# sarahappleby/VAMP

Measured on AMD Instinct MI355X. Metric: walker-steps/sec (log-posterior evals/sec), higher is better.
Workload: dtype f64

## Files before the change

__graft_entry__.py:

```python
import os
import subprocess
import sys

ROOT = os.path.dirname(os.path.abspath(__file__))
if ROOT not in sys.path:
    sys.path.insert(0, ROOT)


def build() -> None:
    from vamp_amd import build as vb
    vb.build()
    subprocess.check_call(["make", "-C", os.path.join(ROOT, "oracle"), "-s"])
    host = os.path.join(ROOT, "tests", "host")
    so = os.path.join(host, "libvoigt_host.so")
    src = os.path.join(host, "voigt_host.cpp")
    hdr = os.path.join(ROOT, "vamp_amd", "csrc", "voigt_math.hpp")
    if not os.path.exists(so) or os.path.getmtime(so) < max(os.path.getmtime(src), os.path.getmtime(hdr)):
        subprocess.check_call(["g++", "-O2", "-std=c++17", "-shared", "-fPIC", "-ffp-contract=off", "-o", so, src])
    pso, psrc = os.path.join(host, "libff_pred_host.so"), os.path.join(host, "ff_pred_host.cpp")
    phdr = os.path.join(ROOT, "vamp_amd", "csrc", "ff_predicates.hpp")
    if not os.path.exists(pso) or os.path.getmtime(pso) < max(os.path.getmtime(psrc), os.path.getmtime(phdr), os.path.getmtime(hdr)):
        subprocess.check_call(["g++", "-O2", "-std=c++17", "-shared", "-fPIC", "-ffp-contract=off", "-o", pso, psrc])
    oso, osrc = os.path.join(host, "libnp_order_host.so"), os.path.join(host, "np_order_host.cpp")
    if not os.path.exists(oso) or os.path.getmtime(oso) < max(os.path.getmtime(osrc), os.path.getmtime(phdr), os.path.getmtime(hdr)):
        subprocess.check_call(["g++", "-O2", "-std=c++17", "-shared", "-fPIC", "-ffp-contract=off", "-o", oso, osrc])
    fake, fsrc = os.path.join(host, "librccl_fake.so"), os.path.join(host, "rccl_fake.cpp")
    if not os.path.exists(fake) or os.path.getmtime(fake) < os.path.getmtime(fsrc):
        subprocess.check_call([os.environ.get("HIPCC", "/opt/rocm/bin/hipcc"), "-O1", "-std=c++17", "-shared", "-fPIC", "-o", fake, fsrc, "-lrt"])
    import vamp_amd
    os.environ.setdefault("VAMP_NO_IMPORT_ORDER_WARNING", "1")
    vamp_amd._lib.load()


def smoke() -> None:
    import numpy as np
    import torch

    import vamp_amd
    from oracle import vamp_oracle as vo

# ... 48 lines not shown
```

vamp_amd/build.py:

```python
import os
import subprocess
import sys

HERE = os.path.dirname(os.path.abspath(__file__))
SRC = os.path.join(HERE, "csrc", "vamp_hip.hip")
OUT = os.path.join(HERE, "libvamp_hip.so")
DEPS = [SRC] + [os.path.join(HERE, "csrc", f) for f in ("ff_matrix.inc", "ff_matrix32.inc", "voigt_math.hpp", "map_search.hpp", "host_plan.hpp",
                                                         "abi_state.hpp", "draws.hpp", "ff_predicates.hpp", "ff_moments.hpp")
                if os.path.exists(os.path.join(HERE, "csrc", f))] + [os.path.join(HERE, "..", "include", "vamp_hip.h")]


FLAGS = ["--offload-arch=gfx950", "-O3", "-std=c++17", "-fno-slp-vectorize", "-shared", "-fPIC"]

SIDE_FLAGS = ["--offload-arch=gfx950", "-O3", "-std=c++17", "-shared", "-fPIC", "-fvisibility=hidden"]
POST_FLAGS = EVID_FLAGS = PRED_FLAGS = LOO_FLAGS = RELABEL_FLAGS = SIDE_FLAGS
SIDE_CALL = os.path.join(HERE, "csrc", "side_call.hpp")
LANE_GROUP = os.path.join(HERE, "csrc", "lane_group.hpp")
CHAIN_GROUPS = os.path.join(HERE, "csrc", "chain_groups.hpp")

DIAG_SRC = os.path.join(HERE, "csrc", "chain_diag.hip")
DIAG_OUT = os.path.join(HERE, "libvamp_diag.so")
DIAG_DEPS = [DIAG_SRC, SIDE_CALL, os.path.join(HERE, "..", "include", "vamp_diag.h")]

POST_SRC = os.path.join(HERE, "csrc", "posterior.hip")
# ... 72 lines not shown
```

vamp_amd/csrc/ff_predicates.hpp:

```cpp
#pragma once
#include "voigt_math.hpp"

namespace vamp {

constexpr double FF_ZONE_MARGIN = 1.0 / 1024.0;

VAMP_DEV bool ff_tile_in_zone(double c, double s, double y, double mid, double half) {
    const double Xf = (fabs(mid - c) + half) * s;
    return fma(Xf, Xf, y * y) < R2_CORE * (1.0 - FF_ZONE_MARGIN);
}

struct NpOrder {
    unsigned long long seq;
    unsigned solo;
    int pairs[4];
};
VAMP_DEV NpOrder np_pair_order(unsigned far, unsigned n6, unsigned n4, unsigned n3) {
    NpOrder o;
    const unsigned cls[4] = {n6, n4 & ~n6, n3 & ~n4, far & ~n3};
    unsigned long long seq = 0ull;
    int sh = 0, last = 0;
    for (int c = 0; c < 4; ++c) {
        for (unsigned m = cls[c]; m; m &= m - 1u) {
            last = __builtin_ctz(m);
// ... 16 lines not shown
```

vamp_amd/csrc/vamp_hip.hip:

```cpp
#include <hip/hip_runtime.h>
#include <dlfcn.h>

#include <algorithm>
#include <atomic>
#include <chrono>
#include <cmath>
#include <cstdint>
#include <cstdio>
#include <cstdlib>
#include <cstring>
#include <new>
#include <string>
#include <vector>

#include "../../include/vamp_hip.h"
#include "abi_state.hpp"
#include "draws.hpp"
#include "host_plan.hpp"
#include "map_search.hpp"
#include "voigt_math.hpp"
#include "ff_predicates.hpp"
#include "ff_moments.hpp"

#ifndef VAMP_EARLY_LOADS
// ... 52 lines not shown
#endif
#ifndef VAMP_WIDE_MAX
#define VAMP_WIDE_MAX 0.75
#endif
#ifndef VAMP_F32_LEAN_STAGE
#define VAMP_F32_LEAN_STAGE 1
#endif
#ifndef VAMP_TILE_MOMENTS
#define VAMP_TILE_MOMENTS 2
#endif
#ifndef VAMP_NODE_PASS
#define VAMP_NODE_PASS 1
#endif
#ifndef VAMP_NP_CLASS_RUNS
#define VAMP_NP_CLASS_RUNS 1
#endif
#ifndef VAMP_TAB_PAIR
#define VAMP_TAB_PAIR 0
#endif
#ifndef VAMP_TILE_HEAD
#define VAMP_TILE_HEAD 0
#endif
namespace {

constexpr int KMAX = 16;
constexpr int KMAX_ALL = VAMP_MAX_COMPONENTS;
static_assert(KMAX_ALL >= KMAX && KMAX_ALL < 64, "lane k stages line k; one spare lane for sd");
constexpr int WAVES_PER_BLOCK = 4;
constexpr long long PACK_MIN_WALKERS = 16384;
constexpr int RES_MAX_MOVERS = 128;
// ... 966 lines not shown
    }
    }
}

#if VAMP_NODE_PASS && VAMP_TILE_MOMENTS != 1 && !VAMP_X_PREFETCH && !defined(VAMP_SKIP_NEAR) && !defined(VAMP_SKIP_FFNODES) && \
    !defined(VAMP_SKIP_CLENSHAW) && !defined(VAMP_SKIP_EXP)
#define VAMP_NODE_PASS_ON 1
#else
#define VAMP_NODE_PASS_ON 0
#endif
#if VAMP_NODE_PASS_ON
__device__ __forceinline__ unsigned ff_fold16(unsigned long long m) {
    const unsigned h = (unsigned)m | (unsigned)(m >> 32);
    return (h | (h >> 16)) & 0xffffu;
}
struct NodeSets { unsigned far, n6, n4, n3, wide; };
template <bool WIDE, bool ZONE, class LDS>
__device__ __forceinline__ void ff_classify_batch_np(const LDS& L, const double2* __restrict__ geo, int K, int lane_, int base, int stride,
                                                     unsigned wide_all, unsigned long long& farmasks, unsigned long long& widemasks,
                                                     unsigned long long& zonemasks, NodeSets& sets, double& mid, double& half) {
    int lane = lane_;
    asm volatile("" : "+v"(lane));
    const int j = lane >> 4, k = lane & (KMAX - 1);
    const double2 g = geo[(base + j * stride) >> 8];
    mid = g.x, half = fabs(g.y);
    const LineRec& me = *reinterpret_cast<const LineRec*>(reinterpret_cast<const char*>(L.line) +
                                                          __umul24((unsigned)(k < K ? k : 0), (unsigned)sizeof(LineRec)));
    const double my_c = me.c, my_s = me.s, my_y = me.y, my_w8 = me.w8, my_wmid = me.wmid;
    const double dist = fabs(mid - my_c) - half;
    const bool my_beyond = (k < K) & (dist >= FF_DIST * half);
    const bool my_far = my_beyond & (dist >= my_w8);
    const double Xe = dist * my_s, r2e = fma(Xe, Xe, my_y * my_y);
    farmasks = __ballot(my_far);
    sets.far = ff_fold16(farmasks);
    sets.n6 = ff_fold16(__ballot(my_far & (r2e < VAMP_FF_R2_M4)));
    sets.n4 = ff_fold16(__ballot(my_far & (r2e < VAMP_FF_R2_M3)));
    sets.n3 = ff_fold16(__ballot(my_far & (r2e < VAMP_FF_R2_M2)));
    widemasks = 0ull;
    if constexpr (WIDE) {
        const bool my_wide = ((((wide_all >> k) & 1u) != 0u) | (VAMP_MID_NODES && (my_beyond & (dist >= my_wmid)))) & !my_far;
        widemasks = __ballot(my_wide);
    }
    sets.wide = ff_fold16(widemasks);
    zonemasks = 0ull;
    if constexpr (ZONE) zonemasks = __ballot(vamp::ff_tile_in_zone(my_c, my_s, my_y, mid, half));
}
constexpr double FF_X_IDLE = 64.0;
static_assert(FF_X_IDLE * FF_X_IDLE >= VAMP_FF_R2_M2 && FF_X_IDLE < vamp::X_FAR, "the idle argument neither deepens a pair nor needs a guard");
template <int M> struct NpDepth { static constexpr int value = M; };
template <bool WIDE, bool GUARD, class LDS>
__device__ __forceinline__ double ff_node_pass(const LDS& L, const double* __restrict__ dct, const double* tab, int lane_, double mid, double half,
                                               unsigned long long farmasks, unsigned long long widemasks, NodeSets sets) {
    int lane = lane_;
    asm volatile("" : "+v"(lane));
    const double xnode = fma(half, dct[FF_MAT + (lane & (FF_NODES - 1))], mid);
    const unsigned far16 = ff_tile_field(farmasks, lane);
    double fs = 0.0;
#if VAMP_NP_CLASS_RUNS
    if (sets.far != 0u) {
    const vamp::NpOrder ord = vamp::np_pair_order(sets.far, sets.n6, sets.n4, sets.n3);
    unsigned long long seq = ord.seq;
    const unsigned far16b = far16 & ~ord.solo;
    struct Pair { double c[2], s[2], y[2], amp[2]; };
    auto read_pair = [&](unsigned long long q) {
        Pair p;
#pragma unroll
        for (int t = 0; t < 2; ++t) {
            const LineRec& ln = L.line[(unsigned)(q >> (4 * t)) & 15u];
            p.c[t] = ln.c, p.s[t] = ln.s, p.y[t] = ln.y, p.amp[t] = ln.amp;
        }
        return p;
    };
// ... 120 lines not shown
                                                        double& chi) {
    if ((lane >> 4) == j) Sx.coef[lane & (FF_NODES - 1)] = a_row;
    const int n = lane & (FF_NODES - 1), g4 = (lane >> 4) * 4;
    const double2* Qr = reinterpret_cast<const double2*>(mt + vamp::FFN_Q + n * FF_NODES + g4);
    const double2 q01 = Qr[0], q23 = Qr[1];
    const double Sv = mt[vamp::FFN_S + n];
    __builtin_amdgcn_wave_barrier();
    const double2* av = reinterpret_cast<const double2*>(Sx.coef + g4);
    const double2 a01 = av[0], a23 = av[1];
    const double a = Sx.coef[n];
    const double acc0 = fma(q01.x, a01.x, 0.5 * Sv), acc1 = q01.y * a01.y;
    const double term = a * (fma(q23.x, a23.x, acc0) + fma(q23.y, a23.y, acc1));
    chi += lane == 0 ? term + c0 : term;
    __builtin_amdgcn_wave_barrier();
}
template <int MODE, class PK, bool TAB, bool WIDE = false, bool GUARD = true>
__device__ __forceinline__ void sweep_range_ff_np(const RegionDev& R, const typename PK::Lds& L, TileScratch& Sx, const double* __restrict__ dct,
                                                  const double* __restrict__ x, const double* __restrict__ f,
                                                  const double* __restrict__ wt, const double* __restrict__ ut,
                                                  const double2* __restrict__ geo, int lane, int base0, int base1, int stride,
                                                  double& chi, const double* tab, unsigned long long wide_all = 0ull,
                                                  const double* __restrict__ mom = nullptr) {
    constexpr int T = TPIX;
    static_assert(PK::LPW == 64 && PK::KCAP <= 16, "far-field tiles: one walker per wavefront, <= 16 lines");
    const int K = R.K;
    const int ntile = base0 < base1 ? (base1 - base0 + stride - 1) / stride : 0;
    const int bfull = __builtin_amdgcn_readfirstlane(base0 + (ntile / FF_BATCH) * (FF_BATCH * stride));
    for (int batch = __builtin_amdgcn_readfirstlane(base0); batch < bfull; batch += FF_BATCH * stride) {
    unsigned long long farmasks, widemasks, zonemasks;
    double fsn;
    {
        NodeSets sets;
        double mid_j, half_j;
        ff_classify_batch_np<WIDE, TAB>(L, geo, K, lane, batch, stride, (unsigned)wide_all, farmasks, widemasks, zonemasks, sets, mid_j, half_j);
        fsn = ff_node_pass<WIDE, GUARD>(L, dct, tab, lane, mid_j, half_j, farmasks, widemasks, sets);
    }
#if VAMP_TILE_MOMENTS == 2
    {
        unsigned long long fm = farmasks, wm = widemasks;
        double a_row = 0.0, amax_row = 0.0;
        bool have_a = false;
#pragma unroll 1
        for (int j = 0; j < FF_BATCH; ++j, fm >>= KMAX, wm >>= KMAX) {
            const unsigned farmask = (unsigned)fm & 0xffffu, widemask = WIDE ? (unsigned)wm & 0xffffu : 0u;
            if ((~(farmask | widemask) & ((1u << K) - 1u)) != 0u) continue;
            const double* mt = mom + ((batch + j * stride) >> 8) * MOM_TILE;
            const double root_c0 = mt[MOM_RC], root_q0 = mt[MOM_RQ];
            if (!vamp::ff_moments_try(root_c0, root_q0)) continue;
            if (!have_a) {
                int eoff = FF_EXP;
                asm volatile("" : "+s"(eoff));
                a_row = -vamp::expm1_taylor_tab(-fsn, dct + eoff);
                amax_row = row16_max(fabs(a_row));
                have_a = true;
            }
            const double amax = __hiloint2double(__builtin_amdgcn_readlane(__double2hiint(amax_row), KMAX * j),
                                                 __builtin_amdgcn_readlane(__double2loint(amax_row), KMAX * j));
            if (!vamp::ff_moments_ok(root_c0, root_q0, amax)) continue;
            ff_moment_chi_nodes_row(Sx, mt, lane_here(), j, a_row, mt[vamp::FFN_C0], chi);
            const unsigned long long field = 0xffffull << (KMAX * j);
            farmasks |= field;
            widemasks |= field;
        }
    }
#endif
#pragma unroll 1
    for (int j = 0; j < FF_BATCH; ++j, farmasks >>= KMAX, widemasks >>= KMAX, zonemasks >>= KMAX) {
        const int base = batch + j * stride;
        double xi[T], tau[T];
#if VAMP_TILE_HEAD
        if ((unsigned)farmasks & (unsigned)widemasks & 0xffffu) continue;
#endif
#pragma unroll
        for (int t = 0; t < T; ++t) {
            xi[t] = x[base + 64 * t + lane];
            tau[t] = 0.0;
        }
#if !VAMP_TILE_HEAD
        if ((unsigned)farmasks & (unsigned)widemasks & 0xffffu) continue;
#endif
        const bool up = __double2hiint(geo[base >> 8].y) >= 0;
        const unsigned farmask = (unsigned)farmasks & 0xffffu;
        const unsigned widemask = WIDE ? (unsigned)widemasks & 0xffffu : 0u;
// ... 39 lines not shown
        int eoff = FF_EXP;
        asm volatile("" : "+s"(eoff));
        const double* ec = dct + eoff;
#pragma unroll
        for (int t = 0; t < T; ++t) {
#if !VAMP_EARLY_LOADS
            fi[t] = f[base + 64 * t + lane];
            wi[t] = wt[base + 64 * t + lane];
#endif
            const double m = vamp::exp_taylor_tab<VAMP_FLUX_EXP_DROP>(-tau[t], ec);
            const double r = (fi[t] - m) * wi[t];
            chi = fma(r, r, chi);
        }
    }
    }
    if (bfull < base1) sweep_range_ff<MODE, PK, TAB, WIDE, GUARD>(R, L, Sx, dct, x, f, wt, ut, geo, lane, bfull, base1, stride, chi, tab, wide_all, mom);
}
#endif
template <int MODE, class PK, bool TAB, bool WIDE, bool GUARD, class... Args>
__device__ __forceinline__ void sweep_range_ff_any(Args&&... args) {
#if VAMP_NODE_PASS_ON
    sweep_range_ff_np<MODE, PK, TAB, WIDE, GUARD>(static_cast<Args&&>(args)...);
#else
    sweep_range_ff<MODE, PK, TAB, WIDE, GUARD>(static_cast<Args&&>(args)...);
#endif
}

#ifndef VAMP_FARFIELD
#define VAMP_FARFIELD 1
#endif

template <int T, int LPW = 64>
__device__ __forceinline__ void tile_w4(float y, const float (&X)[T], float (&H)[T]) {
    float lo = X[0];
#pragma unroll
    for (int t = 1; t < T; ++t) lo = fminf(lo, X[t]);
    lo += y;
// ... 365 lines not shown
                    sweep_range_f32<MODE, PK, 1>(R, L, x, f, wt, lane, from, R.P, PK::LPW, chi);
                }
            }
    } else {
        const double* x = px.x + R.pix_off; const double* f = px.f + R.pix_off; const double* wt = px.wt + R.pix_off;
        if constexpr (VAMP_FARFIELD && PK::FF && MODE != VAMP_GAUSS3 && TPIX == 4) {
            const double* ut = px.u + R.pix_off;
            const double2* geo = px.geo + (R.pix_off >> 8);
            const double* mom = VAMP_TILE_MOMENTS ? px.mom + (R.pix_off >> 8) * MOM_TILE : nullptr;
            const int flags = __builtin_amdgcn_readfirstlane((int)(__double_as_longlong(L.theta[4 * PK::KCAP + 2]) & 0x3ffff));
            const bool guard = (flags >> 16) != 0;
            if constexpr (VAMP_WIDE_NODES && TAB) {
                const unsigned long long wide_all = (unsigned long long)(flags & 0xffff);
                if (VAMP_MID_NODES || wide_all) {
                    if (guard) sweep_range_ff_any<MODE, PK, TAB, true, true>(R, L, Sx, dct, x, f, wt, ut, geo, lane, base0, full, stride, chi, tab, wide_all, mom);
                    else sweep_range_ff_any<MODE, PK, TAB, true, false>(R, L, Sx, dct, x, f, wt, ut, geo, lane, base0, full, stride, chi, tab, wide_all, mom);
                } else {
                    if (guard) sweep_range_ff_any<MODE, PK, TAB, false, true>(R, L, Sx, dct, x, f, wt, ut, geo, lane, base0, full, stride, chi, tab, 0ull, mom);
                    else sweep_range_ff_any<MODE, PK, TAB, false, false>(R, L, Sx, dct, x, f, wt, ut, geo, lane, base0, full, stride, chi, tab, 0ull, mom);
                }
            } else {
                if (guard) sweep_range_ff_any<MODE, PK, TAB, false, true>(R, L, Sx, dct, x, f, wt, ut, geo, lane, base0, full, stride, chi, tab, 0ull, mom);
                else sweep_range_ff_any<MODE, PK, TAB, false, false>(R, L, Sx, dct, x, f, wt, ut, geo, lane, base0, full, stride, chi, tab, 0ull, mom);
            }
        } else if (TPIX > 1) sweep_range<MODE, PK, TPIX, TAB>(R, L, x, f, wt, lane, base0, full, stride, chi, tab);
        if constexpr (PK::TAIL || TPIX == 1)
            if (tail) {
                const int from = TPIX > 1 ? full : 0;
                if constexpr (!PK::FF && TPIX > 1) {
                    const int nt = (R.P - from + PK::LPW - 1) / PK::LPW;
                    if constexpr (TPIX >= 4) { if (nt == 4) sweep_range<MODE, PK, 4, TAB>(R, L, x, f, wt, lane, from, from + 1, 1 << 28, chi, tab); }
                    if constexpr (TPIX >= 3) { if (nt == 3) sweep_range<MODE, PK, 3, TAB>(R, L, x, f, wt, lane, from, from + 1, 1 << 28, chi, tab); }
                    if (nt == 2) sweep_range<MODE, PK, 2, TAB>(R, L, x, f, wt, lane, from, from + 1, 1 << 28, chi, tab);
                    else if (nt == 1) sweep_range<MODE, PK, 1, TAB>(R, L, x, f, wt, lane, from, from + 1, 1 << 28, chi, tab);
                } else {
                    sweep_range<MODE, PK, 1, TAB>(R, L, x, f, wt, lane, from, R.P, PK::LPW, chi, tab);
                }
            }
// ... 235 lines not shown
        for (int d = l; d < R.D; d += PK::LPW) L.theta[d] = theta[w * R.D + d];
    group_barrier<PK>();
    double chi;
    const double v = wave_lnprob<F32, MODE, PK>(R, L, scr[PK::FF ? wave : 0], dct, px, l, &chi, wave, red,
                                                tabs[PK::SPLIT ? 0 : wave].a);
    if (PK::SPLIT && wave != 0) return;
    if (l == 0) {
        lnprob[w] = v;
        if (chi2) chi2[w] = chi;
    }
}

template <int MODE>
__global__ __launch_bounds__(PackSplit::THREADS) void k_dbg_node_sums(const RegionDev* __restrict__ regions, int region, PixPtrs px,
                                                                      const double* __restrict__ theta, double* __restrict__ nodes,
                                                                      unsigned* __restrict__ sets_out) {
    using PK = PackSplit;
    __shared__ typename PK::Lds lds[1];
    __shared__ TileScratch scr[PK::WPB];
    __shared__ alignas(16) double dct[ff_table_doubles<false>()];
    __shared__ LineTables<table_doubles<false, MODE, PK>()> tabs[1];
    ff_fill_table<false>(dct);
    const int wave = threadIdx.x >> 6, lane = threadIdx.x & 63;
    const RegionDev R = regions[region];
    typename PK::Lds& L = lds[0];
    if (wave == 0)
        for (int d = lane; d < R.D; d += 64) L.theta[d] = theta[d];
    group_barrier<PK>();
    const double lp = stage_lines<MODE, PK, true, false, false, true>(R, L, lane, false, wave, tabs[0].a, px.x + R.pix_off);
    if (!(lp > NEG_INF)) return;
    TileScratch& Sx = scr[wave];
    const double* tab = tabs[0].a;
    const double2* geo = px.geo + (R.pix_off >> 8);
    const int flags = __builtin_amdgcn_readfirstlane((int)(__double_as_longlong(L.theta[4 * PK::KCAP + 2]) & 0x3ffff));
    const bool guard = (flags >> 16) != 0;
    const unsigned wide_all = (unsigned)(flags & 0xffff);
    constexpr int TILE = 64 * TPIX;
    const int K = R.K, base1 = (R.P / TILE) * TILE, stride = PARTS * TILE;
    const int base0 = __builtin_amdgcn_readfirstlane(wave * TILE);
    int bfull = base0;
#if VAMP_NODE_PASS_ON
    const int ntile = base0 < base1 ? (base1 - base0 + stride - 1) / stride : 0;
    bfull = __builtin_amdgcn_readfirstlane(base0 + (ntile / FF_BATCH) * (FF_BATCH * stride));
    for (int batch = base0; batch < bfull; batch += FF_BATCH * stride) {
        unsigned long long farmasks, widemasks, zonemasks;
        NodeSets sets;
        double mid, half;
        ff_classify_batch_np<true, true>(L, geo, K, lane, batch, stride, wide_all, farmasks, widemasks, zonemasks, sets, mid, half);
        const double fs = guard ? ff_node_pass<true, true>(L, dct, tab, lane, mid, half, farmasks, widemasks, sets)
                                : ff_node_pass<true, false>(L, dct, tab, lane, mid, half, farmasks, widemasks, sets);
        nodes[((batch + (lane >> 4) * stride) >> 8) * FF_NODES + (lane & (FF_NODES - 1))] = fs;
        if (lane == 0) {
            unsigned* so = sets_out + (batch >> 8) * 5;
            so[0] = sets.far, so[1] = sets.n6, so[2] = sets.n4, so[3] = sets.n3, so[4] = sets.wide;
        }
    }
#endif
    for (int batch = bfull; batch < base1; batch += FF_BATCH * stride) {
        unsigned long long farmasks, widemasks, zonemasks;
        ff_classify_batch<true, false, true>(L, Sx, geo, K, lane, batch, base1, stride, wide_all, farmasks, widemasks, zonemasks);
        for (int j = 0; j < FF_BATCH; ++j, farmasks >>= KMAX, widemasks >>= KMAX) {
            const int base = batch + j * stride;
            if (base >= base1) break;
            const double2 tg = geo[base >> 8];
            const double mid = tg.x, half = fabs(tg.y);
            const int nfar = __builtin_popcount((unsigned)farmasks & 0xffffu), nwide = __builtin_popcount((unsigned)widemasks & 0xffffu);
            const double fs_wide = nwide > 0 ? ff_wide_nodes<typename PK::Lds>(L, Sx.widelist[j], dct, tab, lane, nwide, mid, half) : 0.0;
            const double fs = guard ? ff_node_sums<typename PK::Lds, true>(L, Sx.farlist[j], dct, lane, nfar, mid, half, fs_wide)
                                    : ff_node_sums<typename PK::Lds, false>(L, Sx.farlist[j], dct, lane, nfar, mid, half, fs_wide);
            if (lane < FF_NODES) nodes[(base >> 8) * FF_NODES + lane] = fs;
        }
        __builtin_amdgcn_wave_barrier();
    }
// ... 1204 lines not shown
    HIP_TRY(hipMemcpy(geo_out, c->geo_d.get(), slots * sizeof(double2), hipMemcpyDeviceToHost));
    return slots;
}

long long vampdbg_tile_moments(vamp_ctx* c, double* out) {
    if (!c) return fail(VAMP_ERR_ARG, "vampdbg_tile_moments: bad argument");
    if (c->regions_h.empty()) return fail(VAMP_ERR_STATE, "vampdbg_tile_moments: call vamp_set_regions first");
    if (!VAMP_TILE_MOMENTS || c->f32 || !c->geo_d || !c->mom_d) return 0;
    const long long N = c->regions_h.back().pix_off + c->regions_h.back().P;
    const long long slots = N / (64 * TPIX) + 1;
    HIP_TRY(hipStreamSynchronize(c->stream));
    if (out) HIP_TRY(hipMemcpy(out, c->mom_d.get(), slots * MOM_TILE * sizeof(double), hipMemcpyDeviceToHost));
    return MOM_TILE;
}

long long vampdbg_node_sums(vamp_ctx* c, int region, const double* theta, double* nodes, unsigned* sets) {
    if (!c || !theta || !nodes || !sets) return fail(VAMP_ERR_ARG, "vampdbg_node_sums: bad argument");
    if (c->regions_h.empty()) return fail(VAMP_ERR_STATE, "vampdbg_node_sums: call vamp_set_regions first");
    if (region < 0 || region >= c->n_regions) return fail(VAMP_ERR_ARG, "vampdbg_node_sums: no such region");
    const RegionDev& R = c->regions_h[region];
    const long long tiles = R.P / (64 * TPIX);
    if (c->f32 || c->mode == VAMP_GAUSS3 || !c->geo_d || tiles == 0 || R.K > KMAX) return 0;
    HIP_TRY(hipSetDevice(c->device));
    DevBuf<double> th_d, nodes_d;
    DevBuf<unsigned> sets_d;
    HIP_TRY(th_d.ensure(R.D));
    HIP_TRY(nodes_d.ensure(tiles * FF_NODES));
    HIP_TRY(sets_d.ensure(tiles * 5));
    HIP_TRY(hipMemcpy(th_d.get(), theta, R.D * sizeof(double), hipMemcpyHostToDevice));
    HIP_TRY(hipMemset(nodes_d.get(), 0, tiles * FF_NODES * sizeof(double)));
    HIP_TRY(hipMemset(sets_d.get(), 0xff, tiles * 5 * sizeof(unsigned)));
    HIP_TRY(hipStreamSynchronize(c->stream));
    if (c->mode == VAMP_VOIGT4)
        hipLaunchKernelGGL((k_dbg_node_sums<VAMP_VOIGT4>), dim3(1), dim3(PackSplit::THREADS), 0, c->stream, c->regions_d.get(), region, c->pix(),
                           th_d.get(), nodes_d.get(), sets_d.get());
    else
        hipLaunchKernelGGL((k_dbg_node_sums<VAMP_NBZ3>), dim3(1), dim3(PackSplit::THREADS), 0, c->stream, c->regions_d.get(), region, c->pix(),
                           th_d.get(), nodes_d.get(), sets_d.get());
    HIP_TRY(hipGetLastError());
    HIP_TRY(hipStreamSynchronize(c->stream));
    HIP_TRY(hipMemcpy(nodes, nodes_d.get(), tiles * FF_NODES * sizeof(double), hipMemcpyDeviceToHost));
    HIP_TRY(hipMemcpy(sets, sets_d.get(), tiles * 5 * sizeof(unsigned), hipMemcpyDeviceToHost));
    return tiles;
}

int vamp_version(void) { return VAMP_ABI_VERSION; }

const char* vamp_last_error(void) { return vamp::last_error().c_str(); }

int vamp_device_count(int* n) {
    if (int rc = vamp::check_device_count(n)) return rc;
    HIP_TRY(hipGetDeviceCount(n));
    return VAMP_OK;
}

int vamp_ctx_create(vamp_ctx** out, int device, int dtype, int wofz_kind) {
    if (int rc = vamp::check_ctx_create(out, dtype, wofz_kind)) return rc;
    int ndev = 0;
// ... 642 lines not shown
```

Baseline: 13.75 million.

## Deal adjacent tiles per wave batch and add optional super-tile node pass

Batches in the node pass now cover adjacent tiles rather than tiles strided across waves, with a remainder sweep for leftovers. This groups neighbouring tiles so their line classifications and geometry are similar and can be shared. It also adds a compile-time-disabled super-node pass that evaluates distant lines once on a merged super-tile using a DCT/Chebyshev expansion. The adjacent dealing changes per-wave work distribution and may hurt load balance across waves.

```diff
diff --git a/__graft_entry__.py b/__graft_entry__.py
--- a/__graft_entry__.py
+++ b/__graft_entry__.py
@@ -24,6 +24,10 @@
     oso, osrc = os.path.join(host, "libnp_order_host.so"), os.path.join(host, "np_order_host.cpp")
     if not os.path.exists(oso) or os.path.getmtime(oso) < max(os.path.getmtime(osrc), os.path.getmtime(phdr), os.path.getmtime(hdr)):
         subprocess.check_call(["g++", "-O2", "-std=c++17", "-shared", "-fPIC", "-ffp-contract=off", "-o", oso, osrc])
+    sso, ssrc = os.path.join(host, "libsuper_nodes_host.so"), os.path.join(host, "super_nodes_host.cpp")
+    sinc = os.path.join(ROOT, "vamp_amd", "csrc", "ff_super.inc")
+    if not os.path.exists(sso) or os.path.getmtime(sso) < max(os.path.getmtime(ssrc), os.path.getmtime(phdr), os.path.getmtime(hdr), os.path.getmtime(sinc)):
+        subprocess.check_call(["g++", "-O2", "-std=c++17", "-shared", "-fPIC", "-ffp-contract=off", "-o", sso, ssrc])
     fake, fsrc = os.path.join(host, "librccl_fake.so"), os.path.join(host, "rccl_fake.cpp")
     if not os.path.exists(fake) or os.path.getmtime(fake) < os.path.getmtime(fsrc):
         subprocess.check_call([os.environ.get("HIPCC", "/opt/rocm/bin/hipcc"), "-O1", "-std=c++17", "-shared", "-fPIC", "-o", fake, fsrc, "-lrt"])
diff --git a/vamp_amd/build.py b/vamp_amd/build.py
--- a/vamp_amd/build.py
+++ b/vamp_amd/build.py
@@ -6,7 +6,7 @@
 SRC = os.path.join(HERE, "csrc", "vamp_hip.hip")
 OUT = os.path.join(HERE, "libvamp_hip.so")
 DEPS = [SRC] + [os.path.join(HERE, "csrc", f) for f in ("ff_matrix.inc", "ff_matrix32.inc", "voigt_math.hpp", "map_search.hpp", "host_plan.hpp",
-                                                         "abi_state.hpp", "draws.hpp", "ff_predicates.hpp", "ff_moments.hpp")
+                                                         "abi_state.hpp", "draws.hpp", "ff_predicates.hpp", "ff_moments.hpp", "ff_super.inc")
                 if os.path.exists(os.path.join(HERE, "csrc", f))] + [os.path.join(HERE, "..", "include", "vamp_hip.h")]
 
 
diff --git a/vamp_amd/csrc/ff_predicates.hpp b/vamp_amd/csrc/ff_predicates.hpp
--- a/vamp_amd/csrc/ff_predicates.hpp
+++ b/vamp_amd/csrc/ff_predicates.hpp
@@ -8,6 +8,48 @@
 VAMP_DEV bool ff_tile_in_zone(double c, double s, double y, double mid, double half) {
     const double Xf = (fabs(mid - c) + half) * s;
     return fma(Xf, Xf, y * y) < R2_CORE * (1.0 - FF_ZONE_MARGIN);
+}
+
+#ifndef VAMP_SUPER_DIST
+#define VAMP_SUPER_DIST 4.0
+#endif
+#ifndef VAMP_FF_R2_M3
+#define VAMP_FF_R2_M3 300.0
+#endif
+VAMP_DEV bool ff_super_distant(double c, double s, double y, double Mid, double Half) {
+    const double distS = fabs(Mid - c) - Half;
+    const double Xe = distS * s;
+    return (distS >= VAMP_SUPER_DIST * Half) & (fma(Xe, Xe, y * y) >= VAMP_FF_R2_M3);
+}
+VAMP_DEV double ff_super_r2e(double c, double s, double y, double Mid, double Half) {
+    const double Xe = (fabs(Mid - c) - Half) * s;
+    return fma(Xe, Xe, y * y);
+}
+VAMP_DEV void ff_super_tile(double mid0, double half0, double mid3, double half3, double& Mid, double& Half) {
+    const double lo = fmin(mid0 - half0, mid3 - half3), hi = fmax(mid0 + half0, mid3 + half3);
+    Mid = 0.5 * (lo + hi);
+    Half = 0.5 * (hi - lo);
+}
+
+struct SuperOrder {
+    unsigned long long seq;
+    int n, iters, iters3;
+};
+VAMP_DEV SuperOrder super_order(unsigned dist, unsigned d3) {
+    SuperOrder o;
+    const unsigned cls[2] = {d3 & dist, dist & ~d3};
+    unsigned long long seq = 0ull;
+    int sh = 0;
+    for (int c = 0; c < 2; ++c)
+        for (unsigned m = cls[c]; m; m &= m - 1u) {
+            seq |= (unsigned long long)__builtin_ctz(m) << sh;
+            sh += 4;
+        }
+    o.seq = seq;
+    o.n = sh >> 2;
+    o.iters = (o.n + 7) >> 3;
+    o.iters3 = (__builtin_popcount(cls[0]) + 7) >> 3;
+    return o;
 }
 
 struct NpOrder {
diff --git a/vamp_amd/csrc/ff_super.inc b/vamp_amd/csrc/ff_super.inc
--- /dev/null
+++ b/vamp_amd/csrc/ff_super.inc
@@ -0,0 +1,133 @@
+#ifndef FF_SUPER_QUAL
+#define FF_SUPER_QUAL __device__
+#endif
+FF_SUPER_QUAL const double FF_SUPER_C[256] = {
+    6.25000000000000000e-02, 6.25000000000000000e-02,
+    1.24398090834024616e-01, 1.19617541966526103e-01,
+    1.22598160050403804e-01, 1.03933701537818154e-01,
+    1.19617541966526103e-01, 7.92991605204556860e-02,
+    1.15484941563910842e-01, 4.78354290456362227e-02,
+    1.10240158043544381e-01, 1.22521425411950755e-02,
+    1.03933701537818154e-01, -2.43862902520160345e-02,
+    9.66263066703421242e-02, -5.89245921032497053e-02,
+    8.83883476483184466e-02, -8.83883476483184466e-02,
+    7.92991605204556860e-02, -1.10240158043544381e-01,
+    6.94462791274502722e-02, -1.22598160050403804e-01,
+    5.89245921032497053e-02, -1.24398090834024616e-01,
+    4.78354290456362227e-02, -1.15484941563910842e-01,
+    3.62855846568077983e-02, -9.66263066703421242e-02,
+    2.43862902520160345e-02, -6.94462791274502722e-02,
+    1.22521425411950755e-02, -3.62855846568077983e-02,
+    6.25000000000000000e-02, 6.25000000000000000e-02,
+    1.10240158043544381e-01, 9.66263066703421242e-02,
+    6.94462791274502722e-02, 2.43862902520160345e-02,
+    1.22521425411950755e-02, -5.89245921032497053e-02,
+    -4.78354290456362227e-02, -1.15484941563910842e-01,
+    -9.66263066703421242e-02, -1.19617541966526103e-01,
+    -1.22598160050403804e-01, -6.94462791274502722e-02,
+    -1.19617541966526103e-01, 1.22521425411950755e-02,
+    -8.83883476483184466e-02, 8.83883476483184466e-02,
+    -3.62855846568077983e-02, 1.24398090834024616e-01,
+    2.43862902520160345e-02, 1.03933701537818154e-01,
+    7.92991605204556860e-02, 3.62855846568077983e-02,
+    1.15484941563910842e-01, -4.78354290456362227e-02,
+    1.24398090834024616e-01, -1.10240158043544381e-01,
+    1.03933701537818154e-01, -1.22598160050403804e-01,
+    5.89245921032497053e-02, -7.92991605204556860e-02,
+    6.25000000000000000e-02, 6.25000000000000000e-02,
+    7.92991605204556860e-02, 5.89245921032497053e-02,
+    -2.43862902520160345e-02, -6.94462791274502722e-02,
+    -1.10240158043544381e-01, -1.24398090834024616e-01,
+    -1.15484941563910842e-01, -4.78354290456362227e-02,
+    -3.62855846568077983e-02, 7.92991605204556860e-02,
+    6.94462791274502722e-02, 1.22598160050403804e-01,
+    1.24398090834024616e-01, 3.62855846568077983e-02,
+    8.83883476483184466e-02, -8.83883476483184466e-02,
+    -1.22521425411950755e-02, -1.19617541966526103e-01,
+    -1.03933701537818154e-01, -2.43862902520160345e-02,
+    -1.19617541966526103e-01, 9.66263066703421242e-02,
+    -4.78354290456362227e-02, 1.15484941563910842e-01,
+    5.89245921032497053e-02, 1.22521425411950755e-02,
+    1.22598160050403804e-01, -1.03933701537818154e-01,
+    9.66263066703421242e-02, -1.10240158043544381e-01,
+    6.25000000000000000e-02, 6.25000000000000000e-02,
+    3.62855846568077983e-02, 1.22521425411950755e-02,
+    -1.03933701537818154e-01, -1.22598160050403804e-01,
+    -9.66263066703421242e-02, -3.62855846568077983e-02,
+    4.78354290456362227e-02, 1.15484941563910842e-01,
+    1.24398090834024616e-01, 5.89245921032497053e-02,
+    2.43862902520160345e-02, -1.03933701537818154e-01,
+    -1.10240158043544381e-01, -7.92991605204556860e-02,
+    -8.83883476483184466e-02, 8.83883476483184466e-02,
+    5.89245921032497053e-02, 9.66263066703421242e-02,
+    1.22598160050403804e-01, -6.94462791274502722e-02,
+    1.22521425411950755e-02, -1.10240158043544381e-01,
+    -1.15484941563910842e-01, 4.78354290456362227e-02,
+    -7.92991605204556860e-02, 1.19617541966526103e-01,
+    6.94462791274502722e-02, -2.43862902520160345e-02,
+    1.19617541966526103e-01, -1.24398090834024616e-01,
+    6.25000000000000000e-02, 6.25000000000000000e-02,
+    -1.22521425411950755e-02, -3.62855846568077983e-02,
+    -1.22598160050403804e-01, -1.03933701537818154e-01,
+    3.62855846568077983e-02, 9.66263066703421242e-02,
+    1.15484941563910842e-01, 4.78354290456362227e-02,
+    -5.89245921032497053e-02, -1.24398090834024616e-01,
+    -1.03933701537818154e-01, 2.43862902520160345e-02,
+    7.92991605204556860e-02, 1.10240158043544381e-01,
+    8.83883476483184466e-02, -8.83883476483184466e-02,
+    -9.66263066703421242e-02, -5.89245921032497053e-02,
+    -6.94462791274502722e-02, 1.22598160050403804e-01,
+    1.10240158043544381e-01, -1.22521425411950755e-02,
+    4.78354290456362227e-02, -1.15484941563910842e-01,
+    -1.19617541966526103e-01, 7.92991605204556860e-02,
+    -2.43862902520160345e-02, 6.94462791274502722e-02,
+    1.24398090834024616e-01, -1.19617541966526103e-01,
+    6.25000000000000000e-02, 6.25000000000000000e-02,
+    -5.89245921032497053e-02, -7.92991605204556860e-02,
+    -6.94462791274502722e-02, -2.43862902520160345e-02,
+    1.24398090834024616e-01, 1.10240158043544381e-01,
+    -4.78354290456362227e-02, -1.15484941563910842e-01,
+    -7.92991605204556860e-02, 3.62855846568077983e-02,
+    1.22598160050403804e-01, 6.94462791274502722e-02,
+    -3.62855846568077983e-02, -1.24398090834024616e-01,
+    -8.83883476483184466e-02, 8.83883476483184466e-02,
+    1.19617541966526103e-01, 1.22521425411950755e-02,
+    -2.43862902520160345e-02, -1.03933701537818154e-01,
+    -9.66263066703421242e-02, 1.19617541966526103e-01,
+    1.15484941563910842e-01, -4.78354290456362227e-02,
+    -1.22521425411950755e-02, -5.89245921032497053e-02,
+    -1.03933701537818154e-01, 1.22598160050403804e-01,
+    1.10240158043544381e-01, -9.66263066703421242e-02,
+    6.25000000000000000e-02, 6.25000000000000000e-02,
+    -9.66263066703421242e-02, -1.10240158043544381e-01,
+    2.43862902520160345e-02, 6.94462791274502722e-02,
+    5.89245921032497053e-02, -1.22521425411950755e-02,
+    -1.15484941563910842e-01, -4.78354290456362227e-02,
+    1.19617541966526103e-01, 9.66263066703421242e-02,
+    -6.94462791274502722e-02, -1.22598160050403804e-01,
+    -1.22521425411950755e-02, 1.19617541966526103e-01,
+    8.83883476483184466e-02, -8.83883476483184466e-02,
+    -1.24398090834024616e-01, 3.62855846568077983e-02,
+    1.03933701537818154e-01, 2.43862902520160345e-02,
+    -3.62855846568077983e-02, -7.92991605204556860e-02,
+    -4.78354290456362227e-02, 1.15484941563910842e-01,
+    1.10240158043544381e-01, -1.24398090834024616e-01,
+    -1.22598160050403804e-01, 1.03933701537818154e-01,
+    7.92991605204556860e-02, -5.89245921032497053e-02,
+    6.25000000000000000e-02, 6.25000000000000000e-02,
+    -1.19617541966526103e-01, -1.24398090834024616e-01,
+    1.03933701537818154e-01, 1.22598160050403804e-01,
+    -7.92991605204556860e-02, -1.19617541966526103e-01,
+    4.78354290456362227e-02, 1.15484941563910842e-01,
+    -1.22521425411950755e-02, -1.10240158043544381e-01,
+    -2.43862902520160345e-02, 1.03933701537818154e-01,
+    5.89245921032497053e-02, -9.66263066703421242e-02,
+    -8.83883476483184466e-02, 8.83883476483184466e-02,
+    1.10240158043544381e-01, -7.92991605204556860e-02,
+    -1.22598160050403804e-01, 6.94462791274502722e-02,
+    1.24398090834024616e-01, -5.89245921032497053e-02,
+    -1.15484941563910842e-01, 4.78354290456362227e-02,
+    9.66263066703421242e-02, -3.62855846568077983e-02,
+    -6.94462791274502722e-02, 2.43862902520160345e-02,
+    3.62855846568077983e-02, -1.22521425411950755e-02,
+};
diff --git a/vamp_amd/csrc/vamp_hip.hip b/vamp_amd/csrc/vamp_hip.hip
--- a/vamp_amd/csrc/vamp_hip.hip
+++ b/vamp_amd/csrc/vamp_hip.hip
@@ -90,6 +90,12 @@
 #endif
 #ifndef VAMP_NP_CLASS_RUNS
 #define VAMP_NP_CLASS_RUNS 1
+#endif
+#ifndef VAMP_DEAL_ADJ
+#define VAMP_DEAL_ADJ 1
+#endif
+#ifndef VAMP_SUPER_NODES
+#define VAMP_SUPER_NODES 0
 #endif
 #ifndef VAMP_TAB_PAIR
 #define VAMP_TAB_PAIR 0
@@ -1086,11 +1092,19 @@
     const unsigned h = (unsigned)m | (unsigned)(m >> 32);
     return (h | (h >> 16)) & 0xffffu;
 }
+#if VAMP_SUPER_NODES && VAMP_DEAL_ADJ
+#define VAMP_SUPER_ON 1
+#include "ff_super.inc"
+struct NodeSets { unsigned far, n6, n4, n3, wide, dist, d3; double Mid, Half; };
+#else
+#define VAMP_SUPER_ON 0
 struct NodeSets { unsigned far, n6, n4, n3, wide; };
+#endif
 template <bool WIDE, bool ZONE, class LDS>
 __device__ __forceinline__ void ff_classify_batch_np(const LDS& L, const double2* __restrict__ geo, int K, int lane_, int base, int stride,
                                                      unsigned wide_all, unsigned long long& farmasks, unsigned long long& widemasks,
-                                                     unsigned long long& zonemasks, NodeSets& sets, double& mid, double& half) {
+                                                     unsigned long long& zonemasks, NodeSets& sets, double& mid, double& half,
+                                                     bool super_ok = false) {
     int lane = lane_;
     asm volatile("" : "+v"(lane));
     const int j = lane >> 4, k = lane & (KMAX - 1);
@@ -1116,18 +1130,109 @@
     sets.wide = ff_fold16(widemasks);
     zonemasks = 0ull;
     if constexpr (ZONE) zonemasks = __ballot(vamp::ff_tile_in_zone(my_c, my_s, my_y, mid, half));
+#if VAMP_SUPER_ON
+    sets.dist = sets.d3 = 0u;
+    sets.Mid = sets.Half = 0.0;
+    if (super_ok) {
+        const double2 g0 = geo[base >> 8], g3 = geo[(base + (FF_BATCH - 1) * stride) >> 8];
+        vamp::ff_super_tile(g0.x, fabs(g0.y), g3.x, fabs(g3.y), sets.Mid, sets.Half);
+        const bool my_dist = (k < K) & vamp::ff_super_distant(my_c, my_s, my_y, sets.Mid, sets.Half);
+        const bool my_d3 = my_dist & (vamp::ff_super_r2e(my_c, my_s, my_y, sets.Mid, sets.Half) < VAMP_FF_R2_M2);
+        const unsigned all4 = (unsigned)farmasks & (unsigned)(farmasks >> 16) & (unsigned)(farmasks >> 32) & (unsigned)(farmasks >> 48) & 0xffffu;
+        sets.dist = (unsigned)__ballot(my_dist) & all4;
+        sets.d3 = (unsigned)__ballot(my_d3) & sets.dist;
+        sets.far &= ~sets.dist, sets.n6 &= ~sets.dist, sets.n4 &= ~sets.dist, sets.n3 &= ~sets.dist;
+    }
+#endif
 }
 constexpr double FF_X_IDLE = 64.0;
 static_assert(FF_X_IDLE * FF_X_IDLE >= VAMP_FF_R2_M2 && FF_X_IDLE < vamp::X_FAR, "the idle argument neither deepens a pair nor needs a guard");
 template <int M> struct NpDepth { static constexpr int value = M; };
+#if VAMP_SUPER_ON
+template <class LDS>
+__device__ __forceinline__ double ff_super_pass(const LDS& L, TileScratch& Sx, const double* __restrict__ dct, int lane, double xnode,
+                                                const NodeSets& sets) {
+    const vamp::SuperOrder ord = vamp::super_order(sets.dist, sets.d3);
+    const int n = lane & (FF_NODES - 1), g4 = (lane >> 4) * 4;
+    const double xs = fma(sets.Half, dct[FF_MAT + n], sets.Mid);
+    unsigned long long seq = ord.seq;
+    int left = ord.n;
+    double acc = 0.0;
+    auto run = [&](auto depth, int iters) {
+        constexpr int M = decltype(depth)::value;
+#pragma unroll 1
+        for (int i = 0; i < iters; ++i) {
+            const unsigned s32 = (unsigned)seq >> g4;
+            double X[2], y[2], amp[2], r2[2], nn[2], d[2];
+#pragma unroll
+            for (int t = 0; t < 2; ++t) {
+                const LineRec& ln = *reinterpret_cast<const LineRec*>(reinterpret_cast<const char*>(L.line) +
+                                                                      __umul24((s32 >> (16 * t)) & 15u, (unsigned)sizeof(LineRec)));
+                const bool live = (g4 >> 2) + 4 * t < left;
+                const double Xl = fabs(xs - ln.c) * ln.s;
+                X[t] = live ? Xl : FF_X_IDLE;
+                y[t] = ln.y;
+                amp[t] = live ? ln.amp : 0.0;
+                r2[t] = fma(X[t], X[t], y[t] * y[t]);
+                vamp::voigt_jfrac_nd<M>(X[t], y[t], r2[t], nn[t], d[t], vamp::GHFrac<M>::Z, vamp::GHFrac<M>::C);
+            }
+            const double ra = vamp::rcp_nr(d[0] * d[1]);
+            acc = fma(amp[0], nn[0] * (ra * d[1]), acc);
+            acc = fma(amp[1], nn[1] * (ra * d[0]), acc);
+            seq >>= 32;
+            left -= 8;
+        }
+    };
+    run(NpDepth<3>{}, ord.iters3);
+    run(NpDepth<2>{}, ord.iters - ord.iters3);
+    {
+        const int me = lane_here();
+        const int a16 = (me ^ 16) << 2, a32 = (me ^ 32) << 2;
+        acc += __hiloint2double(__builtin_amdgcn_ds_bpermute(a16, __double2hiint(acc)), __builtin_amdgcn_ds_bpermute(a16, __double2loint(acc)));
+        acc += __hiloint2double(__builtin_amdgcn_ds_bpermute(a32, __double2hiint(acc)), __builtin_amdgcn_ds_bpermute(a32, __double2loint(acc)));
+    }
+    if (lane < FF_NODES) Sx.coef[lane] = acc;
+    __builtin_amdgcn_wave_barrier();
+    const double2* crow = reinterpret_cast<const double2*>(FF_SUPER_C) + n;
+    const double2* fv = reinterpret_cast<const double2*>(Sx.coef);
+    double a0 = 0.0, a1 = 0.0;
+#pragma unroll
+    for (int n2 = 0; n2 < FF_NODES / 2; ++n2) {
+        const double2 m = crow[n2 * FF_NODES], f2 = fv[n2];
+        a0 = fma(m.x, f2.x, a0);
+        a1 = fma(m.y, f2.y, a1);
+    }
+    __builtin_amdgcn_wave_barrier();
+    if (lane < FF_NODES) Sx.coef[lane] = a0 + a1;
+    __builtin_amdgcn_wave_barrier();
+    const double t = (xnode - sets.Mid) * vamp::rcp_nr(sets.Half), t2 = t + t;
+    double b1 = 0.0, b2 = 0.0;
+#pragma unroll
+    for (int k = FF_NODES - 1; k >= 1; --k) {
+        const double b = fma(t2, b1, Sx.coef[k] - b2);
+        b2 = b1;
+        b1 = b;
+    }
+    const double p = fma(t, b1, Sx.coef[0] - b2);
+    __builtin_amdgcn_wave_barrier();
+    return p;
+}
+#endif
 template <bool WIDE, bool GUARD, class LDS>
 __device__ __forceinline__ double ff_node_pass(const LDS& L, const double* __restrict__ dct, const double* tab, int lane_, double mid, double half,
-                                               unsigned long long farmasks, unsigned long long widemasks, NodeSets sets) {
+                                               unsigned long long farmasks, unsigned long long widemasks, NodeSets sets,
+                                               TileScratch* Sx = nullptr) {
     int lane = lane_;
     asm volatile("" : "+v"(lane));
     const double xnode = fma(half, dct[FF_MAT + (lane & (FF_NODES - 1))], mid);
+    double fs = 0.0;
+#if VAMP_SUPER_ON
+    if (sets.dist != 0u) {
+        fs = ff_super_pass(L, *Sx, dct, lane, xnode, sets);
+        farmasks &= ~(sets.dist * 0x0001000100010001ull);
+    }
+#endif
     const unsigned far16 = ff_tile_field(farmasks, lane);
-    double fs = 0.0;
 #if VAMP_NP_CLASS_RUNS
     if (sets.far != 0u) {
     const vamp::NpOrder ord = vamp::np_pair_order(sets.far, sets.n6, sets.n4, sets.n3);
@@ -1278,7 +1383,7 @@
     chi += lane == 0 ? term + c0 : term;
     __builtin_amdgcn_wave_barrier();
 }
-template <int MODE, class PK, bool TAB, bool WIDE = false, bool GUARD = true>
+template <int MODE, class PK, bool TAB, bool WIDE = false, bool GUARD = true, bool SUPER = false>
 __device__ __forceinline__ void sweep_range_ff_np(const RegionDev& R, const typename PK::Lds& L, TileScratch& Sx, const double* __restrict__ dct,
                                                   const double* __restrict__ x, const double* __restrict__ f,
                                                   const double* __restrict__ wt, const double* __restrict__ ut,
@@ -1289,15 +1394,30 @@
     static_assert(PK::LPW == 64 && PK::KCAP <= 16, "far-field tiles: one walker per wavefront, <= 16 lines");
     const int K = R.K;
     const int ntile = base0 < base1 ? (base1 - base0 + stride - 1) / stride : 0;
+#if VAMP_DEAL_ADJ
+    (void)ntile;
+    const int tstride = 64 * T, bstep = FF_BATCH * stride;
+    const int bfull = __builtin_amdgcn_readfirstlane((base1 / bstep) * bstep);
+    const int bfirst = FF_BATCH * base0, brest = bfull + base0;
+#else
+    const int tstride = stride, bstep = FF_BATCH * stride;
     const int bfull = __builtin_amdgcn_readfirstlane(base0 + (ntile / FF_BATCH) * (FF_BATCH * stride));
-    for (int batch = __builtin_amdgcn_readfirstlane(base0); batch < bfull; batch += FF_BATCH * stride) {
+    const int bfirst = base0, brest = bfull;
+#endif
+    for (int batch = __builtin_amdgcn_readfirstlane(bfirst); batch < bfull; batch += bstep) {
     unsigned long long farmasks, widemasks, zonemasks;
     double fsn;
     {
         NodeSets sets;
         double mid_j, half_j;
-        ff_classify_batch_np<WIDE, TAB>(L, geo, K, lane, batch, stride, (unsigned)wide_all, farmasks, widemasks, zonemasks, sets, mid_j, half_j);
+#if VAMP_SUPER_ON
+        ff_classify_batch_np<WIDE, TAB>(L, geo, K, lane, batch, tstride, (unsigned)wide_all, farmasks, widemasks, zonemasks, sets, mid_j, half_j,
+                                        SUPER);
+        fsn = ff_node_pass<WIDE, GUARD>(L, dct, tab, lane, mid_j, half_j, farmasks, widemasks, sets, &Sx);
+#else
+        ff_classify_batch_np<WIDE, TAB>(L, geo, K, lane, batch, tstride, (unsigned)wide_all, farmasks, widemasks, zonemasks, sets, mid_j, half_j);
         fsn = ff_node_pass<WIDE, GUARD>(L, dct, tab, lane, mid_j, half_j, farmasks, widemasks, sets);
+#endif
     }
 #if VAMP_TILE_MOMENTS == 2
     {
@@ -1308,7 +1428,7 @@
         for (int j = 0; j < FF_BATCH; ++j, fm >>= KMAX, wm >>= KMAX) {
             const unsigned farmask = (unsigned)fm & 0xffffu, widemask = WIDE ? (unsigned)wm & 0xffffu : 0u;
             if ((~(farmask | widemask) & ((1u << K) - 1u)) != 0u) continue;
-            const double* mt = mom + ((batch + j * stride) >> 8) * MOM_TILE;
+            const double* mt = mom + ((batch + j * tstride) >> 8) * MOM_TILE;
             const double root_c0 = mt[MOM_RC], root_q0 = mt[MOM_RQ];
             if (!vamp::ff_moments_try(root_c0, root_q0)) continue;
             if (!have_a) {
@@ -1330,7 +1450,7 @@
 #endif
 #pragma unroll 1
     for (int j = 0; j < FF_BATCH; ++j, farmasks >>= KMAX, widemasks >>= KMAX, zonemasks >>= KMAX) {
-        const int base = batch + j * stride;
+        const int base = batch + j * tstride;
         double xi[T], tau[T];
 #if VAMP_TILE_HEAD
         if ((unsigned)farmasks & (unsigned)widemasks & 0xffffu) continue;
@@ -1400,13 +1520,17 @@
         }
     }
     }
-    if (bfull < base1) sweep_range_ff<MODE, PK, TAB, WIDE, GUARD>(R, L, Sx, dct, x, f, wt, ut, geo, lane, bfull, base1, stride, chi, tab, wide_all, mom);
-}
-#endif
-template <int MODE, class PK, bool TAB, bool WIDE, bool GUARD, class... Args>
+    if (brest < base1) sweep_range_ff<MODE, PK, TAB, WIDE, GUARD>(R, L, Sx, dct, x, f, wt, ut, geo, lane, brest, base1, stride, chi, tab, wide_all, mom);
+}
+#endif
+#ifndef VAMP_SUPER_ON
+#define VAMP_SUPER_ON 0
+#endif
+template <int MODE, class PK, bool TAB, bool WIDE, bool GUARD, bool SUPER = false, class... Args>
 __device__ __forceinline__ void sweep_range_ff_any(Args&&... args) {
 #if VAMP_NODE_PASS_ON
-    sweep_range_ff_np<MODE, PK, TAB, WIDE, GUARD>(static_cast<Args&&>(args)...);
+    static_assert(!(SUPER && GUARD), "a guard walker keeps the ordinary pass");
+    sweep_range_ff_np<MODE, PK, TAB, WIDE, GUARD, SUPER && VAMP_SUPER_ON>(static_cast<Args&&>(args)...);
 #else
     sweep_range_ff<MODE, PK, TAB, WIDE, GUARD>(static_cast<Args&&>(args)...);
 #endif
@@ -1802,14 +1926,16 @@
                 const unsigned long long wide_all = (unsigned long long)(flags & 0xffff);
                 if (VAMP_MID_NODES || wide_all) {
                     if (guard) sweep_range_ff_any<MODE, PK, TAB, true, true>(R, L, Sx, dct, x, f, wt, ut, geo, lane, base0, full, stride, chi, tab, wide_all, mom);
+                    else if (VAMP_SUPER_ON && wide_all == 0ull)
+                        sweep_range_ff_any<MODE, PK, TAB, true, false, true>(R, L, Sx, dct, x, f, wt, ut, geo, lane, base0, full, stride, chi, tab, wide_all, mom);
                     else sweep_range_ff_any<MODE, PK, TAB, true, false>(R, L, Sx, dct, x, f, wt, ut, geo, lane, base0, full, stride, chi, tab, wide_all, mom);
                 } else {
                     if (guard) sweep_range_ff_any<MODE, PK, TAB, false, true>(R, L, Sx, dct, x, f, wt, ut, geo, lane, base0, full, stride, chi, tab, 0ull, mom);
-                    else sweep_range_ff_any<MODE, PK, TAB, false, false>(R, L, Sx, dct, x, f, wt, ut, geo, lane, base0, full, stride, chi, tab, 0ull, mom);
+                    else sweep_range_ff_any<MODE, PK, TAB, false, false, true>(R, L, Sx, dct, x, f, wt, ut, geo, lane, base0, full, stride, chi, tab, 0ull, mom);
                 }
             } else {
                 if (guard) sweep_range_ff_any<MODE, PK, TAB, false, true>(R, L, Sx, dct, x, f, wt, ut, geo, lane, base0, full, stride, chi, tab, 0ull, mom);
-                else sweep_range_ff_any<MODE, PK, TAB, false, false>(R, L, Sx, dct, x, f, wt, ut, geo, lane, base0, full, stride, chi, tab, 0ull, mom);
+                else sweep_range_ff_any<MODE, PK, TAB, false, false, true>(R, L, Sx, dct, x, f, wt, ut, geo, lane, base0, full, stride, chi, tab, 0ull, mom);
             }
         } else if (TPIX > 1) sweep_range<MODE, PK, TPIX, TAB>(R, L, x, f, wt, lane, base0, full, stride, chi, tab);
         if constexpr (PK::TAIL || TPIX == 1)
@@ -2075,8 +2201,9 @@
 template <int MODE>
 __global__ __launch_bounds__(PackSplit::THREADS) void k_dbg_node_sums(const RegionDev* __restrict__ regions, int region, PixPtrs px,
                                                                       const double* __restrict__ theta, double* __restrict__ nodes,
-                                                                      unsigned* __restrict__ sets_out) {
+                                                                      unsigned* __restrict__ sets_out, bool adj_) {
     using PK = PackSplit;
+    const bool adj = VAMP_DEAL_ADJ && adj_;
     __shared__ typename PK::Lds lds[1];
     __shared__ TileScratch scr[PK::WPB];
     __shared__ alignas(16) double dct[ff_table_doubles<false>()];
@@ -2099,25 +2226,28 @@
     constexpr int TILE = 64 * TPIX;
     const int K = R.K, base1 = (R.P / TILE) * TILE, stride = PARTS * TILE;
     const int base0 = __builtin_amdgcn_readfirstlane(wave * TILE);
-    int bfull = base0;
+    int bfull = base0, brest = base0;
 #if VAMP_NODE_PASS_ON
     const int ntile = base0 < base1 ? (base1 - base0 + stride - 1) / stride : 0;
-    bfull = __builtin_amdgcn_readfirstlane(base0 + (ntile / FF_BATCH) * (FF_BATCH * stride));
-    for (int batch = base0; batch < bfull; batch += FF_BATCH * stride) {
+    const int tstride = adj ? TILE : stride, bstep = FF_BATCH * stride;
+    bfull = __builtin_amdgcn_readfirstlane(adj ? (base1 / bstep) * bstep : base0 + (ntile / FF_BATCH) * bstep);
+    brest = adj ? bfull + base0 : bfull;
+    for (int batch = adj ? FF_BATCH * base0 : base0; batch < bfull; batch += bstep) {
         unsigned long long farmasks, widemasks, zonemasks;
         NodeSets sets;
         double mid, half;
-        ff_classify_batch_np<true, true>(L, geo, K, lane, batch, stride, wide_all, farmasks, widemasks, zonemasks, sets, mid, half);
+        ff_classify_batch_np<true, true>(L, geo, K, lane, batch, tstride, wide_all, farmasks, widemasks, zonemasks, sets, mid, half,
+                                         adj && !guard && wide_all == 0u);
         const double fs = guard ? ff_node_pass<true, true>(L, dct, tab, lane, mid, half, farmasks, widemasks, sets)
-                                : ff_node_pass<true, false>(L, dct, tab, lane, mid, half, farmasks, widemasks, sets);
-        nodes[((batch + (lane >> 4) * stride) >> 8) * FF_NODES + (lane & (FF_NODES - 1))] = fs;
+                                : ff_node_pass<true, false>(L, dct, tab, lane, mid, half, farmasks, widemasks, sets, &Sx);
+        nodes[((batch + (lane >> 4) * tstride) >> 8) * FF_NODES + (lane & (FF_NODES - 1))] = fs;
         if (lane == 0) {
             unsigned* so = sets_out + (batch >> 8) * 5;
             so[0] = sets.far, so[1] = sets.n6, so[2] = sets.n4, so[3] = sets.n3, so[4] = sets.wide;
         }
     }
 #endif
-    for (int batch = bfull; batch < base1; batch += FF_BATCH * stride) {
+    for (int batch = brest; batch < base1; batch += FF_BATCH * stride) {
         unsigned long long farmasks, widemasks, zonemasks;
         ff_classify_batch<true, false, true>(L, Sx, geo, K, lane, batch, base1, stride, wide_all, farmasks, widemasks, zonemasks);
         for (int j = 0; j < FF_BATCH; ++j, farmasks >>= KMAX, widemasks >>= KMAX) {
@@ -3352,7 +3482,7 @@
     return MOM_TILE;
 }
 
-long long vampdbg_node_sums(vamp_ctx* c, int region, const double* theta, double* nodes, unsigned* sets) {
+static long long dbg_node_sums(vamp_ctx* c, int region, const double* theta, double* nodes, unsigned* sets, bool adj) {
     if (!c || !theta || !nodes || !sets) return fail(VAMP_ERR_ARG, "vampdbg_node_sums: bad argument");
     if (c->regions_h.empty()) return fail(VAMP_ERR_STATE, "vampdbg_node_sums: call vamp_set_regions first");
     if (region < 0 || region >= c->n_regions) return fail(VAMP_ERR_ARG, "vampdbg_node_sums: no such region");
@@ -3371,15 +3501,23 @@
     HIP_TRY(hipStreamSynchronize(c->stream));
     if (c->mode == VAMP_VOIGT4)
         hipLaunchKernelGGL((k_dbg_node_sums<VAMP_VOIGT4>), dim3(1), dim3(PackSplit::THREADS), 0, c->stream, c->regions_d.get(), region, c->pix(),
-                           th_d.get(), nodes_d.get(), sets_d.get());
+                           th_d.get(), nodes_d.get(), sets_d.get(), adj);
     else
         hipLaunchKernelGGL((k_dbg_node_sums<VAMP_NBZ3>), dim3(1), dim3(PackSplit::THREADS), 0, c->stream, c->regions_d.get(), region, c->pix(),
-                           th_d.get(), nodes_d.get(), sets_d.get());
+                           th_d.get(), nodes_d.get(), sets_d.get(), adj);
     HIP_TRY(hipGetLastError());
     HIP_TRY(hipStreamSynchronize(c->stream));
     HIP_TRY(hipMemcpy(nodes, nodes_d.get(), tiles * FF_NODES * sizeof(double), hipMemcpyDeviceToHost));
     HIP_TRY(hipMemcpy(sets, sets_d.get(), tiles * 5 * sizeof(unsigned), hipMemcpyDeviceToHost));
     return tiles;
+}
+int vampdbg_super_nodes(void) { return VAMP_SUPER_ON; }
+long long vampdbg_node_sums(vamp_ctx* c, int region, const double* theta, double* nodes, unsigned* sets) {
+    return dbg_node_sums(c, region, theta, nodes, sets, false);
+}
+long long vampdbg_node_sums_adj(vamp_ctx* c, int region, const double* theta, double* nodes, unsigned* sets) {
+    if (!(VAMP_DEAL_ADJ && VAMP_NODE_PASS_ON)) return 0;
+    return dbg_node_sums(c, region, theta, nodes, sets, true);
 }
 
 int vamp_version(void) { return VAMP_ABI_VERSION; }
```

Result: faster. 13.97 million (median of 6 runs) (+1.6%).
